# stefantaubert/waveglow

Measured on AMD Instinct MI355X. Metric: audio samples/sec/GPU (22.05 kHz) WaveGlow-256 infer; real-time factor, higher is better.
Workload: dtype f16 MFMA operands, f32 accumulate/flow state, fp16 I/O; 1 GPU; configs[1]: 256ch WaveGlow.infer, batch=16/GPU mels 80x864, fp16 I/O, sigma=0.6; parallelism=utterance-sharded x1, no collective

## Files before the change

### waveglow_amd/csrc/api.cpp

```cpp
#include <hip/hip_runtime.h>

#include <cmath>
#include <cstdarg>
#include <cstdio>
#include <cstdlib>
#include <cstring>
#include <map>
#include <string>
#include <vector>

#include "../../include/waveglow_amd.h"
#include "wg_common.h"

using namespace wg;

namespace {

thread_local std::string g_err;

int fail(int code, const char* fmt, ...) {
  char buf[512];
  va_list ap;
  va_start(ap, fmt);
  vsnprintf(buf, sizeof buf, fmt, ap);
// ... 57 lines not shown
constexpr float kSigmScale = -1.4426950408889634f;

struct LayerOffsets {
  size_t wA1, bias1, wA2, bias2, wEs;
  size_t wA1f = 0;
  size_t wA1x = 0, wA1fx = 0;
};
struct FlowOffsets {
  std::vector<LayerOffsets> layers;
  size_t wstart, bstart, out_init, winv, wfwd;
  size_t wStA = 0;
  int c, h;
  double logdet;
};

}

struct wg_handle {
  wg_config cfg;
  int device;
  int NS;
  std::vector<int> c_k;
  std::vector<std::string> expected;
  std::map<std::string, HostTensor> tensors;
  bool finalized = false;
  char* d_blob = nullptr;
  size_t blob_bytes = 0;
  char* d_cond = nullptr;
  char* d_cond16 = nullptr;
  size_t cond_layer_bytes = 0, cond_flow_bytes = 0;
  std::vector<FlowOffsets> flows;
  int n_cu = 256;
  int force_bn = 0;
  bool fold_start = true;
  unsigned long long* dbg_stamps = nullptr;
  bool prof = false;
  unsigned prof_mask = ~0u;
  std::vector<hipEvent_t> ev;
  std::vector<int> ev_class;
  size_t ev_used = 0;
  double prof_ms[8] = {0, 0, 0, 0, 0, 0, 0, 0};
  int64_t prof_n[8] = {0, 0, 0, 0, 0, 0, 0, 0};
  hipStream_t aux[3] = {nullptr, nullptr, nullptr};
  std::vector<hipEvent_t> sync_ev;
  size_t sync_next = 0;
  hipEvent_t mark_ev[16] = {nullptr, nullptr, nullptr, nullptr, nullptr, nullptr, nullptr, nullptr,
                            nullptr, nullptr, nullptr, nullptr, nullptr, nullptr, nullptr, nullptr};
  static constexpr int kPins = 4;
  void* pin[kPins] = {nullptr, nullptr, nullptr, nullptr};
  size_t pin_bytes[kPins] = {0, 0, 0, 0};
  hipEvent_t pin_ev[kPins] = {nullptr, nullptr, nullptr, nullptr};
  int pin_next = 0;
};

namespace {

std::vector<int> flow_channels(const wg_config& c) {
  std::vector<int> out;
  int rem = c.n_group;
  for (int k = 0; k < c.n_flows; ++k) {
    if (k % c.n_early_every == 0 && k > 0) rem -= c.n_early_size;
    out.push_back(rem);
  }
  return out;
}

// ... 147 lines not shown
}

extern "C" {

const char* wg_version(void) { return "waveglow_amd 0.1 (gfx950)"; }
const char* wg_last_error(void) { return g_err.c_str(); }

int wg_create(const wg_config* cfg, int device_id, wg_handle** out) {
  if (!cfg || !out) return fail(WG_ERR_INVALID, "null argument");
  const wg_config& c = *cfg;
  if (c.n_group != 8) return fail(WG_ERR_INVALID, "n_group=%d unsupported (only 8)", c.n_group);
  if (c.kernel_size != 3) return fail(WG_ERR_INVALID, "kernel_size=%d unsupported (only 3)", c.kernel_size);
  if (c.n_channels != 64 && c.n_channels != 128 && c.n_channels != 256 && c.n_channels != 512)
    return fail(WG_ERR_INVALID, "n_channels=%d unsupported (64, 128, 256, 512)", c.n_channels);
  if (c.n_layers < 1 || c.n_layers > 10) return fail(WG_ERR_INVALID, "n_layers=%d unsupported (1..10)", c.n_layers);
  if (c.upsample_kernel != 1024 || c.upsample_stride != 256)
    return fail(WG_ERR_INVALID, "upsample geometry %d/%d unsupported (1024/256)", c.upsample_kernel, c.upsample_stride);
  if (c.n_mel_channels < 16 || c.n_mel_channels > 80 || c.n_mel_channels % 16 != 0)
    return fail(WG_ERR_INVALID, "n_mel_channels=%d unsupported (multiple of 16, <= 80)", c.n_mel_channels);
  if (c.n_flows < 1 || c.n_early_every < 1 || c.n_early_size < 0 || c.n_early_size % 2 != 0)
    return fail(WG_ERR_INVALID, "bad flow configuration");
  std::vector<int> ck = flow_channels(c);
  if (ck.back() < 2 || ck.back() % 2 != 0) return fail(WG_ERR_INVALID, "flow configuration leaves %d channels", ck.back());
  wg_handle* h = new wg_handle();
  h->cfg = c;
  h->device = device_id;
  {
    int ncu = 0;
    if (hipDeviceGetAttribute(&ncu, hipDeviceAttributeMultiprocessorCount, device_id) == hipSuccess && ncu > 0) h->n_cu = ncu;
  }
  h->NS = c.n_mel_channels * c.n_group;
  h->c_k = ck;
  if (const char* e = getenv("WG_FORCE_BN")) h->force_bn = atoi(e);
  if (const char* e = getenv("WG_NO_START_FOLD")) h->fold_start = !(*e == '1');
  h->expected.push_back("upsample.weight");
  h->expected.push_back("upsample.bias");
  for (int k = 0; k < c.n_flows; ++k) {
    const std::string ks = std::to_string(k);
    h->expected.push_back("convinv." + ks + ".conv.weight");
    const std::string p = "WN." + ks + ".";
    for (const char* n : {"start", "cond_layer", "end"}) {
      h->expected.push_back(p + n + ".weight");
      h->expected.push_back(p + n + ".bias");
    }
    for (int i = 0; i < c.n_layers; ++i) {
      const std::string is = std::to_string(i);
      h->expected.push_back(p + "in_layers." + is + ".weight");
      h->expected.push_back(p + "in_layers." + is + ".bias");
      h->expected.push_back(p + "res_skip_layers." + is + ".weight");
      h->expected.push_back(p + "res_skip_layers." + is + ".bias");
    }
  }
  *out = h;
  return WG_OK;
}

int wg_destroy(wg_handle* h) {
  if (!h) return WG_OK;
  if (h->d_blob) hipFree(h->d_blob);
  if (h->d_cond) hipFree(h->d_cond);
  if (h->d_cond16) hipFree(h->d_cond16);
  for (hipEvent_t e : h->ev) hipEventDestroy(e);
  for (hipEvent_t e : h->sync_ev) hipEventDestroy(e);
  for (hipEvent_t e : h->mark_ev)
    if (e) hipEventDestroy(e);
  for (int i = 0; i < wg_handle::kPins; ++i) {
// ... 328 lines not shown
  return carve(h, g, nullptr).bytes;
}

size_t wg_forward_workspace_bytes(const wg_handle* h, int32_t B, int32_t n_frames, int32_t audio_len) {
  if (!h || B < 1 || n_frames < 1 || audio_len < h->cfg.n_group || audio_len % h->cfg.n_group) return 0;
  RowGeom g = make_geom(h->cfg, B, audio_len / h->cfg.n_group, n_frames);
  return carve(h, g, nullptr).bytes;
}

static int run_wn(wg_handle* h, int k, const RowGeom& g, Workspace& w, _Float16*& cur, _Float16*& oth, hipStream_t s) {
  const wg_config& c = h->cfg;
  const int C = c.n_channels;
  int BN = wn_block_n(C);
  if (BN == 128) {
    const int64_t t128 = (int64_t)kPhases * (g.Rp / 128), ncu = h->n_cu > 0 ? h->n_cu : 1;
    const int64_t r128 = (t128 + ncu - 1) / ncu, r64 = (2 * t128 + ncu - 1) / ncu;
    if (t128 < 4 * ncu && 6 * r64 < 10 * r128) BN = 64;
  }
  if (BN == 128 && h->force_bn == 64) BN = 64;
  if (h->force_bn == 128 && wn_block_n(C) == 128) BN = 128;
  const FlowOffsets& fo = h->flows[k];
  for (int i = 0; i < c.n_layers; ++i) {
    const LayerOffsets& lo = fo.layers[i];
    WnLayerArgs a;
    a.x_in = cur;
    a.x_out = oth;
    const bool fold0 = (i == 0) && h->fold_start;
    a.x_tap = fold0 ? w.A0 : cur;
    a.x_chunks_per_tap = fold0 ? 1 : C / 64;
    a.melT = w.melT;
    a.frag16 = wn_frag16(C, BN) ? 1 : 0;
    a.wStA = fold0 && wn_res_a0(C) ? (const _Float16*)(h->d_blob + fo.wStA) : nullptr;
    a.a0_fold = fold0 ? 1 : 0;
    a.wA1c = (const _Float16*)((a.frag16 ? h->d_cond16 : h->d_cond) + h->cond_flow_bytes * k + h->cond_layer_bytes * i);
    a.wA1 = (const _Float16*)(h->d_blob + (a.frag16 ? (fold0 ? lo.wA1fx : lo.wA1x) : (fold0 ? lo.wA1f : lo.wA1)));
    a.bias1 = (const float*)(h->d_blob + lo.bias1);
    a.wA2 = (const _Float16*)(h->d_blob + lo.wA2);
    a.bias2 = (const float*)(h->d_blob + lo.bias2);
    a.wEs = (const _Float16*)(h->d_blob + lo.wEs);
    a.out = w.OUT;
    a.g = g;
    a.dil = 1 << i;
    a.n_cond_steps = c.n_mel_channels / 16;
    a.M = c.n_mel_channels;
    a.has_res = i < c.n_layers - 1;
    a.row0 = 0;
    a.tiles_per_phase = g.Rp / BN;
    a.sp = nullptr;
    a.save_t = a.save_s = a.save_a = nullptr;
    a.in0 = a.in1 = nullptr;
    a.out0 = nullptr;
    a.n_tiles = kPhases * a.tiles_per_phase;
    a.stamps = h->dbg_stamps;
    a.n_cu = h->n_cu;
    {
      Prof p(h, s, 2);
      HIP_TRY(launch_wn_layer(a, C, BN, s));
    }
    WG_DBG(s, "wn_layer");
    if (a.has_res) std::swap(cur, oth);
  }
  return WG_OK;
}

int wg_infer(wg_handle* h, const void* mel, const void* z_init, const void* const* z_early, int32_t n_z_early,
             float sigma, void* audio, int32_t B, int32_t n_frames, int32_t io_dtype, void* workspace,
// ... 278 lines not shown
```

### waveglow_amd/csrc/kernels.hip

```cpp
#include "wg_common.h"

#include <cstdlib>
#include <type_traits>

namespace wg {

typedef _Float16 half8 __attribute__((ext_vector_type(8)));
typedef _Float16 half4 __attribute__((ext_vector_type(4)));
typedef float f32x16 __attribute__((ext_vector_type(16)));
typedef float f32x4 __attribute__((ext_vector_type(4)));

#define WG_GPTR(p) ((const __attribute__((address_space(1))) void*)(p))
#define WG_LPTR(p) ((__attribute__((address_space(3))) void*)(p))

__device__ __forceinline__ float load_io(const void* p, size_t i, int f16) {
  return f16 ? (float)((const _Float16*)p)[i] : ((const float*)p)[i];
}

__device__ __forceinline__ float gate_act(float u, float v) {
  const float e1 = __builtin_amdgcn_exp2f(__builtin_amdgcn_fmed3f(u, -60.0f, 60.0f));
  const float t = 1.0f + __builtin_amdgcn_exp2f(v);
  return (e1 - 1.0f) * __builtin_amdgcn_rcpf(fmaf(e1, t, t));
}

__device__ __forceinline__ void gate_act3(float u, float v, float& th, float& sg, float& ac) {
  const float e1 = __builtin_amdgcn_exp2f(__builtin_amdgcn_fmed3f(u, -60.0f, 60.0f));
  const float t = 1.0f + __builtin_amdgcn_exp2f(__builtin_amdgcn_fmed3f(v, -60.0f, 60.0f));
  const float r = __builtin_amdgcn_rcpf(fmaf(e1, t, t));
  ac = fmaf(e1, r, -r);
  sg = fmaf(e1, r, r);
  th = ac * t;
}

__device__ __forceinline__ void glds16(const void* sbase, unsigned voff, unsigned lds_addr) {
  unsigned keep;
  asm volatile("s_mov_b32 %0, m0\n\ts_mov_b32 m0, %3\n\ts_nop 2\n\tglobal_load_lds_dwordx4 %1, %2\n\ts_mov_b32 m0, %0"
               : "=&s"(keep) : "v"(voff), "s"(sbase), "s"(lds_addr) : "memory");
}
template <int OFF>
__device__ __forceinline__ void gload16(half8& dst, const void* sbase, unsigned voff) {
  asm volatile("s_nop 4\n\tglobal_load_dwordx4 %0, %1, %2 offset:%3" : "=v"(dst) : "v"(voff), "s"(sbase), "i"(OFF) : "memory");
}

#ifdef WG_STAMPS
#define WG_STAMP(i)                                                                              \
  do {                                                                                           \
    __builtin_amdgcn_sched_barrier(0);                                                           \
    unsigned long long _t;                                                                       \
    asm volatile("s_memtime %0\n\ts_waitcnt lgkmcnt(0)" : "=s"(_t)::"memory");                   \
    if (a.stamps && HAS_RES && tid == 0) a.stamps[(size_t)tile * 8 + (i)] = _t;                        \
    __builtin_amdgcn_sched_barrier(0);                                                           \
  } while (0)
#else
#define WG_STAMP(i) do {} while (0)
#endif

constexpr bool kPersistent = true;
#ifdef WG_DBG_NO_XTILE_DMA
constexpr bool kXTileDMA = false;
#else
constexpr bool kXTileDMA = kPersistent;
#endif
constexpr int kTilesPerWG = 2;
#ifdef WG_NO_PIPE_EPI
constexpr bool kPipeEpi = false;
#else
constexpr bool kPipeEpi = true;
#endif

#ifdef WG_NO_PRIO
constexpr bool kPrio = false;
#else
constexpr bool kPrio = true;
#endif
// ... 7 lines not shown
#else
constexpr bool kQ2Late = true;
#endif
#ifdef WG_NO_DEEP_Q2
constexpr bool kDeepQ2 = false;
#else
constexpr bool kDeepQ2 = true;
#endif
#ifdef WG_NO_WES_LDS
constexpr bool kWesLds = false;
#else
constexpr bool kWesLds = true;
#endif
#ifdef WG_NO_DEEP
constexpr bool kDeep = false;
#else
constexpr bool kDeep = true;
#endif

__device__ __forceinline__ void mfma16_acc(f32x4& c, const half8& a, const half8& b) {
  c = __builtin_amdgcn_mfma_f32_16x16x32_f16(a, b, c, 0, 0, 0);
}

template <int C> struct WnCfg {
  static constexpr int NW = (C >= 256) ? 8 : C / 32;
  static constexpr int BN = (C >= 512) ? 64 : 128;
};

template <int N> __device__ __forceinline__ void wait_vm() {
  asm volatile("s_waitcnt vmcnt(%0)" :: "i"(N) : "memory");
  __builtin_amdgcn_sched_barrier(0);
}

template <int C, int NW, int BN, bool HAS_RES, int TPW, int CX, int MODE = 0, int NTAPS = 3, bool HAS_COND = true, bool DEEP = false, bool M16 = false>
__global__ void __launch_bounds__(NW * 64) wn_layer_kernel(const WnLayerArgs a) {
  constexpr bool TR = MODE == 1;
  constexpr bool PLAIN = MODE >= 2;
  constexpr int MB = C / (32 * NW);
  constexpr int MT = PLAIN ? MB : 2 * MB;
  constexpr int NTHREADS = NW * 64;
  constexpr int NT = BN / 32;
  constexpr int CC = CX;
  constexpr int NKX = NTAPS * CC;
  constexpr int BT_BYTES = BN * 128;
  constexpr int ACT_ROW = 2 * C + 16;
  constexpr int K2 = C / 16;
  constexpr int NG = BN * 8 / NTHREADS;
  constexpr int NAH = MT * 2;
  constexpr bool DEFER = (MB == 1);
  static_assert(BN * 8 % NTHREADS == 0 && MB >= 1 && MB <= 2 && NKX >= 1 && (NTAPS == 1 || NTAPS == 3), "tile geometry");
  constexpr bool Q2L = !M16 && kQ2Late && DEFER && !DEEP && (NG + NT - 1) / NT == 1 && NT >= NG + MT;
  static_assert(!M16 || (MODE == 0 && MB == 1 && DEFER && !DEEP && NT >= 2), "16x16x32 variant");
  constexpr bool A0G = MODE == 0 && CX == 1 && NTAPS == 1;
  static_assert(!DEEP || (MODE == 0 && DEFER && HAS_COND && MT <= NT && NG <= NT && ((NKX >= 4 && NKX % 2 == 0) || NKX == 1)), "deep prefetch variant");
  static_assert(MODE == 0 || (TPW == 1 && CX == ((MODE == 2 || MODE == 4) ? 2 : 1) * (C / 64)) || (MODE == 3 && CX == 1), "training variants");

  extern __shared__ __attribute__((aligned(16))) char smem[];
  char* const sB = smem;
  char* const sActs = MODE == 4 ? smem : smem + 2 * BT_BYTES;

  const int tid = threadIdx.x;
  const int wave = __builtin_amdgcn_readfirstlane(tid >> 6);
  int lane = tid & 63, ln = lane & 31, lh = lane >> 5;

  unsigned pvoff[NG];
  int pchunk[NG];
  int swB;
  int l15 = lane & 15, l4 = lane >> 4;
  unsigned a_voff;
  auto set_lane_ids = [&]() {
    int t = tid;
    asm volatile("" : "+v"(t));
    lane = t & 63;
    ln = lane & 31;
    lh = lane >> 5;
    swB = M16 ? (lane >> 1) & 7 : (ln >> 1) & 7;
    l15 = lane & 15;
    l4 = lane >> 4;
    a_voff = lane * 16;
#pragma unroll
    for (int i = 0; i < NG; ++i) {
      const int idx = i * NTHREADS + t;
      const int row = idx >> 3, pc = idx & 7;
      pchunk[i] = pc ^ ((row >> 1) & 7);
      pvoff[i] = row * 128 + (pchunk[i] << 4);
    }
  };
  set_lane_ids();
  const unsigned sB_addr = (unsigned)(size_t)WG_LPTR(sB);
  const int R = a.g.R, Rp = a.g.Rp, Fp = a.g.Fp, M = a.M;
  const int nK = NKX + (HAS_COND ? a.n_cond_steps : 0);
  const int mel_rows_per_utt = a.g.T + 6;

  auto xstep_src = [&](int p, int jt, int ks) -> const char* {
    const int tap = ks / CC, cc = ks - tap * CC;
    const int pp = p + (tap - NTAPS / 2) * a.dil;
    const int row = kRowPad + (pp & 31) * Rp + a.row0 + jt * BN + (pp >> 5);
    return (const char*)(a.x_tap + ((size_t)cc * R + row) * 64);
  };
  auto sp_src = [&](int p, int jt, int s_) -> const char* {
    const int row = kRowPad + p * Rp + a.row0 + jt * BN;
    return (const char*)(a.sp + ((size_t)s_ * R + row) * 64);
  };
  int mrow[NG];
  auto cond_voff = [&](int s, int i) -> unsigned {
    const int k0 = s * 64 + pchunk[i] * 8;
    const int j = (k0 >= M) + (k0 >= 2 * M) + (k0 >= 3 * M);
    return (unsigned)(((mrow[i] - j) * M + (k0 - j * M)) * 2);
  };
  auto stage_B_piece = [&](int p, int jt, int ks, int bufsel, int i) {
#ifndef WG_DBG_NO_DMA
    const unsigned lds = __builtin_amdgcn_readfirstlane(sB_addr + bufsel * BT_BYTES + (i * NTHREADS + wave * 64) * 16);
    if constexpr (A0G) {
      if (ks < NKX) {
        const int row = (i * NTHREADS + tid) >> 3, lc = pchunk[i];
        const int pp = p + ((lc < 3 ? lc : 1) - 1) * a.dil;
        const unsigned prow = (unsigned)(kRowPad + (pp & 31) * Rp + a.row0 + jt * BN + (pp >> 5) + row);
        glds16(a.x_tap, prow * 128u + (lc < 3 ? 0u : (unsigned)lc * 16u), lds);
        return;
      }
    }
    if (ks < NKX) glds16(xstep_src(p, jt, ks), pvoff[i], lds);
    else if constexpr (MODE != 0) glds16(sp_src(p, jt, ks - NKX), pvoff[i], lds);
    else glds16(a.melT, cond_voff(ks - NKX, i), lds);
#endif
  };
  auto read_B = [&](const char* buf, int nt, int k16) -> half8 {
#ifdef WG_DBG_NO_LDSREAD
    half8 z; asm volatile("" : "=v"(z)); return z;
#endif
    const int n = nt * 32 + ln;
    const int c = (k16 * 2 + lh) ^ swB;
    return *(const half8*)(buf + n * 128 + c * 16);
  };
  auto read_B16 = [&](const char* buf, int g, int nt) -> half8 {
    const int n = (NT * (g & 1) + nt) * 16 + l15;
    const int c = (4 * (g >> 1) + l4) ^ swB;
    return *(const half8*)(buf + n * 128 + c * 16);
  };
  const char* wA1c_p = nullptr;
  auto load_Aq = [&](int ks, int g, int mt, half8& dst) {
    const char* base = ks < NKX ? (const char*)a.wA1 : wA1c_p;
    const int kl = ks < NKX ? ks : ks - NKX;
    const char* p = base + ((size_t)(2 * kl + (g >> 1)) * NW + wave) * (NAH * 1024) + (mt * 2 + (g & 1)) * 1024;
#ifndef WG_DBG_NO_ALOAD
    gload16<0>(dst, p, a_voff);
#else
    asm volatile("" : "=v"(dst));
#endif
  };
  auto load_A16 = [&](int ks, int s_, int m, half8& dst) {
    const char* base = ks < NKX ? (const char*)a.wA1 : wA1c_p;
    const int kl = ks < NKX ? ks : ks - NKX;
#ifndef WG_DBG_NO_ALOAD
    gload16<0>(dst, base + ((size_t)(2 * kl + s_) * NW + wave) * (NAH * 1024) + m * 1024, a_voff);
#else
    asm volatile("" : "=v"(dst));
#endif
  };
  int tile_b0 = 0;
  const bool fp_ge_bn = Fp >= BN;
  auto column_of = [&](int rr, int p, int& b, int& t) -> bool {
    int rem = rr - tile_b0 * Fp;
    b = tile_b0;
    if (fp_ge_bn) {
      if (rem >= Fp) { rem -= Fp; ++b; }
    } else {
      const int qd = rem / Fp;
      b += qd;
      rem -= qd * Fp;
    }
    const int fq = rem - a.g.Gf;
    t = fq * 32 + p;
    if (!(b < a.g.B && fq >= 0 && fq < a.g.F && t < a.g.L)) return false;
    return a.g.frames == nullptr || t < 32 * a.g.frames[b];
  };

  int tile, tile_end;
  const int tile_step = gridDim.x >> 3;
  int run_start, run_quarter = 0;
  {
    const int bid = blockIdx.x, ntl = a.n_tiles;
    const int xcd = bid & 7, idx = bid >> 3;
    const int qq = ntl >> 3, r = ntl & 7;
    const int start = xcd < r ? xcd * (qq + 1) : r * (qq + 1) + (xcd - r) * qq;
    tile_end = start + (xcd < r ? qq + 1 : qq);
    tile = start + idx;
    run_start = start;
// ... 23 lines not shown
#pragma unroll
  for (int it = 0; it < TPW; ++it, tile += tile_step) {
    if (tile >= tile_end) break;
    if (it > 0) set_lane_ids();
    const int tile_m = tile_of(tile);
    const int p = tile_m / a.tiles_per_phase;
    const int jt = tile_m - p * a.tiles_per_phase;
    const int rr0 = a.row0 + jt * BN;
    tile_b0 = rr0 / Fp;
    const int r0 = kRowPad + p * Rp + rr0;
    const int next_tile = tile + tile_step;
    wA1c_p = (const char*)a.wA1c + (MODE != 0 ? (size_t)0 : (size_t)p * (2 * a.n_cond_steps) * NW * (NAH * 1024));
    if constexpr (!kXTileDMA) {
      if (it > 0) {
#pragma unroll
        for (int i = 0; i < NG; ++i) stage_B_piece(p, jt, 0, par, i);
      }
    }
    half8 Q[DEEP ? 2 : 1][4][MT];
    if constexpr (DEEP) {
#pragma unroll
      for (int g = 0; g < 4; ++g)
#pragma unroll
        for (int mt = 0; mt < MT; ++mt) load_Aq(0, g, mt, Q[0][g][mt]);
#pragma unroll
      for (int g = 0; g < (kDeepQ2 ? 2 : 3); ++g)
#pragma unroll
        for (int mt = 0; mt < MT; ++mt) load_Aq(1, g, mt, Q[DEEP ? 1 : 0][g][mt]);
    } else {
#pragma unroll
      for (int g = 0; g < (Q2L || M16 ? 2 : 3); ++g)
#pragma unroll
        for (int mt = 0; mt < MT; ++mt) {
          if constexpr (M16) load_A16(0, 0, 2 * g + mt, q[g][mt]);
          else load_Aq(0, g, mt, q[g][mt]);
        }
    }
    if constexpr (MODE == 0) {
#pragma unroll
      for (int i = 0; i < NG; ++i) {
        int b, t;
        const int rr = rr0 + ((i * NTHREADS + tid) >> 3);
        const bool ok = column_of(rr, p, b, t);
        mrow[i] = ok ? 3 + b * mel_rows_per_utt + 3 + (t >> 5) : 3;
      }
    }
    unsigned vmask = 0;
#pragma unroll
    for (int nt = 0; nt < NT; ++nt) {
      int cb, ct;
      vmask |= column_of(rr0 + nt * 32 + ln, p, cb, ct) ? (1u << nt) : 0u;
    }
    WG_STAMP(0);
    f32x16 acc[MT][NT];
    f32x4 acc4[M16 ? MT : 1][M16 ? NT : 1][4];
    auto acc_at = [&](int mt, int nt, int e) -> float {
      if constexpr (M16) return acc4[mt][nt][e >> 2][e & 3];
      else return acc[mt][nt][e];
    };
#pragma unroll
    for (int mt = 0; mt < MT; ++mt) {
      f32x16 v;
      if constexpr (PLAIN) {
#pragma unroll
        for (int j = 0; j < 16; ++j) v[j] = 0.0f;
      } else {
        const int row0 = (mt < MB ? 0 : C) + (wave * MB + (mt < MB ? mt : mt - MB)) * 32;
// ... 25 lines not shown
    constexpr int LPS = (MT + NT - 1) / NT;
    constexpr int GPS = (NG + NT - 1) / NT;
    half8 bf[2][NT];
    constexpr bool PRIO = kPrio && NW == 8 && ((BN == 128 && ((MODE == 0 && CX == C / 64) || MODE == 1)) || (C == 512 && MODE == 0 && CX == C / 64));
    auto prio_set = [&](int hi_grp) {
      if (hi_grp == 1)
        asm volatile("s_cmp_lt_u32 %0, 4\n\ts_cbranch_scc1 .Lpa%=\n\ts_setprio 1\n\ts_branch .Lpb%=\n.Lpa%=:\n\ts_setprio 0\n.Lpb%=:" :: "s"(wave) : "memory", "scc");
      else
        asm volatile("s_cmp_lt_u32 %0, 4\n\ts_cbranch_scc1 .Lpa%=\n\ts_setprio 0\n\ts_branch .Lpb%=\n.Lpa%=:\n\ts_setprio 1\n.Lpb%=:" :: "s"(wave) : "memory", "scc");
    };
    auto mfma_col = [&](int g, int nt) {
      if constexpr (M16) {
        const int t16 = NT * (g & 1) + nt;
#pragma unroll
        for (int m = 0; m < 4; ++m) {
          mfma16_acc(acc4[m >> 1][t16 >> 1][2 * (m & 1) + (t16 & 1)], q[2 * (g >> 1) + (m >> 1)][m & 1], bf[g & 1][nt]);
        }
      } else {
#pragma unroll
        for (int mt = 0; mt < MT; ++mt) {
#ifdef WG_DBG_MFMA16
          f32x4 lo = __builtin_shufflevector(acc[mt][nt], acc[mt][nt], 0, 1, 2, 3);
          f32x4 hi = __builtin_shufflevector(acc[mt][nt], acc[mt][nt], 4, 5, 6, 7);
          lo = __builtin_amdgcn_mfma_f32_16x16x32_f16(q[g][mt], bf[g & 1][nt], lo, 0, 0, 0);
          hi = __builtin_amdgcn_mfma_f32_16x16x32_f16(q[g][mt], bf[g & 1][nt], hi, 0, 0, 0);
#pragma unroll
          for (int j = 0; j < 4; ++j) { acc[mt][nt][j] = lo[j]; acc[mt][nt][4 + j] = hi[j]; }
#else
          acc[mt][nt] = __builtin_amdgcn_mfma_f32_32x32x16_f16(q[g][mt], bf[g & 1][nt], acc[mt][nt], 0, 0, 0);
#endif
        }
      }
    };
    auto kstep = [&](auto more_tag, auto ncond_tag, auto first_tag, int ks) {
      constexpr bool more = decltype(more_tag)::value;
      constexpr bool ncond = decltype(ncond_tag)::value;
      constexpr bool first = decltype(first_tag)::value;
      const char* buf = sB + ((ks + par) & 1) * BT_BYTES;
      const char* src_next = nullptr;
      if constexpr (more && !ncond) src_next = xstep_src(p, jt, ks + 1);
      if constexpr (more && ncond && MODE != 0) src_next = sp_src(p, jt, ks + 1 - NKX);
      const unsigned lds_next = sB_addr + ((ks + 1 + par) & 1) * BT_BYTES + wave * 1024;
#pragma unroll
      for (int nt = 0; nt < NT; ++nt) bf[0][nt] = M16 ? read_B16(buf, 0, nt) : read_B(buf, nt, 0);
      __builtin_amdgcn_sched_barrier(0);
      auto dma_slot = [&](int nt) {
        if constexpr (more) {
#pragma unroll
          for (int i = nt * GPS; i < (nt + 1) * GPS && i < NG; ++i) {
#ifndef WG_DBG_NO_DMA
            const unsigned lds = __builtin_amdgcn_readfirstlane(lds_next + i * NTHREADS * 16);
            if constexpr (ncond && MODE == 0) glds16(a.melT, cond_voff(ks + 1 - NKX, i), lds);
            else glds16(src_next, pvoff[i], lds);
#endif
          }
        }
      };
      if constexpr (PRIO) {
        prio_set(1);
        __builtin_amdgcn_sched_barrier(0);
      }
      if constexpr (DEFER) {
#pragma unroll
        for (int nt = 0; nt < NT; ++nt) {
          if constexpr (!first) mfma_col(3, nt);
          __builtin_amdgcn_sched_barrier(0);
          dma_slot(nt);
          if constexpr (Q2L) {
            if (nt >= NG && nt - NG < MT) load_Aq(ks, 2, nt - NG, q[2][nt - NG]);
          }
          __builtin_amdgcn_sched_barrier(0);
        }
      }
#pragma unroll
      for (int g = 0; g < (DEFER ? 3 : 4); ++g) {
        if constexpr (M16) {
          if (g == 0) wait_vm<more ? NG : 0>();
          if (g == 2) wait_vm<0>();
        } else {
        if (g == 1) wait_vm<more ? 2 * MT + NG : 2 * MT>();
        if (g == 2) wait_vm<Q2L ? (more ? 2 * MT : MT) : (more ? NG + 2 * MT : MT)>();
        if (g == 3) wait_vm<more ? 2 * MT : 0>();
        }
#pragma unroll
        for (int nt = 0; nt < NT; ++nt) {
          mfma_col(g, nt);
          __builtin_amdgcn_sched_barrier(0);
          if (g < 3) bf[(g + 1) & 1][nt] = M16 ? read_B16(buf, g + 1, nt) : read_B(buf, nt, g + 1);
          if (!DEFER && g == 0) dma_slot(nt);
          if constexpr (M16) {
            constexpr int LP16 = (4 + NT - 1) / NT;
            if (g == 0 || (g == 2 && more)) {
#pragma unroll
              for (int m = nt * LP16; m < (nt + 1) * LP16 && m < 4; ++m)
                load_A16(g == 0 ? ks : ks + 1, g == 0 ? 1 : 0, m, q[(g == 0 ? 2 : 0) + (m >> 1)][m & 1]);
            }
          } else if (g == 0 || more) {
#pragma unroll
            for (int mt = nt * LPS; mt < (nt + 1) * LPS && mt < MT; ++mt)
              load_Aq(g == 0 ? ks : ks + 1, (g + 3) & 3, mt, q[(g + 3) & 3][mt]);
          }
          if constexpr (PRIO) {
            if (g == 0 && nt == NT - 1) prio_set(0);
          }
          __builtin_amdgcn_sched_barrier(0);
        }
      }
      if constexpr (more) {
        if constexpr (DEFER && !Q2L && !M16) {
#pragma unroll
          for (int mt = 0; mt < MT; ++mt) load_Aq(ks + 1, 2, mt, q[2][mt]);
        }
        asm volatile("s_waitcnt vmcnt(%0) lgkmcnt(0)" :: "i"(M16 ? 4 : Q2L ? MT : 2 * MT) : "memory");
#ifndef WG_DBG_NO_BARRIER
        __builtin_amdgcn_s_barrier();
#endif
        __builtin_amdgcn_sched_barrier(0);
      }
    };
    auto kstep_d = [&](auto par_tag, auto more_tag, auto more2_tag, auto ncond_tag, auto first_tag, int ks) {
      constexpr int P = DEEP ? decltype(par_tag)::value : 0, PO = DEEP ? 1 - P : 0;
      constexpr bool more = decltype(more_tag)::value, more2 = decltype(more2_tag)::value;
      constexpr bool ncond = decltype(ncond_tag)::value, first = decltype(first_tag)::value;
      const char* buf = sB + ((ks + par) & 1) * BT_BYTES;
      const char* src_next = nullptr;
      if constexpr (more && !ncond) src_next = xstep_src(p, jt, ks + 1);
      const unsigned lds_next = sB_addr + ((ks + 1 + par) & 1) * BT_BYTES + wave * 1024;
#pragma unroll
// ... 55 lines not shown
      using P1 = std::integral_constant<int, 1>;
      if constexpr (NKX == 1) {
        kstep_d(P0{}, T_{}, T_{}, T_{}, T_{}, 0);
        kstep_d(P1{}, T_{}, T_{}, T_{}, F_{}, 1);
        kstep_d(P0{}, T_{}, T_{}, T_{}, F_{}, 2);
        kstep_d(P1{}, T_{}, T_{}, T_{}, F_{}, 3);
        kstep_d(P0{}, T_{}, F_{}, T_{}, F_{}, 4);
        kstep_d(P1{}, F_{}, F_{}, F_{}, F_{}, 5);
      } else {
        kstep_d(P0{}, T_{}, T_{}, F_{}, T_{}, 0);
#pragma clang loop unroll(disable)
        for (int ks = 1; ks < NKX - 1; ks += 2) {
          kstep_d(P1{}, T_{}, T_{}, F_{}, F_{}, ks);
          kstep_d(P0{}, T_{}, T_{}, F_{}, F_{}, ks + 1);
        }
        kstep_d(P1{}, T_{}, T_{}, T_{}, F_{}, NKX - 1);
        kstep_d(P0{}, T_{}, T_{}, T_{}, F_{}, NKX);
        kstep_d(P1{}, T_{}, T_{}, T_{}, F_{}, NKX + 1);
        kstep_d(P0{}, T_{}, T_{}, T_{}, F_{}, NKX + 2);
        kstep_d(P1{}, T_{}, F_{}, T_{}, F_{}, NKX + 3);
        kstep_d(P0{}, F_{}, F_{}, F_{}, F_{}, NKX + 4);
      }
      constexpr int PL = (NKX + 4) & 1;
      wait_vm<0>();
#pragma unroll
      for (int nt = 0; nt < NT; ++nt)
#pragma unroll
        for (int mt = 0; mt < MT; ++mt)
          acc[mt][nt] = __builtin_amdgcn_mfma_f32_32x32x16_f16(Q[DEEP ? PL : 0][3][mt], bf[1][nt], acc[mt][nt], 0, 0, 0);
    }
    if constexpr (!DEEP) {
      using T_ = std::true_type;
      using F_ = std::false_type;
      if constexpr (NKX == 1) {
        if constexpr (HAS_COND) kstep(T_{}, T_{}, T_{}, 0);
        else kstep(F_{}, F_{}, T_{}, 0);
      } else {
        kstep(T_{}, F_{}, T_{}, 0);
#pragma clang loop unroll(disable)
        for (int ks = 1; ks < NKX - 1; ++ks) kstep(T_{}, F_{}, F_{}, ks);
        if constexpr (HAS_COND) kstep(T_{}, T_{}, F_{}, NKX - 1);
        else kstep(F_{}, F_{}, F_{}, NKX - 1);
      }
      if constexpr (HAS_COND) {
#pragma clang loop unroll(disable)
        for (int ks = NKX; ks < nK - 1; ++ks) kstep(T_{}, T_{}, F_{}, ks);
        kstep(F_{}, F_{}, F_{}, nK - 1);
      }
    }
    if constexpr (DEFER && !DEEP) {
      wait_vm<0>();
#pragma unroll
      for (int nt = 0; nt < NT; ++nt) mfma_col(3, nt);
    }
    if constexpr (PRIO) asm volatile("s_setprio 0" ::: "memory");
    __builtin_amdgcn_sched_barrier(0);
    par = (par + nK) & 1;
    if constexpr (kXTileDMA) {
      if (next_tile < tile_end) {
        const int tn = tile_of(next_tile), pn = tn / a.tiles_per_phase;
#pragma unroll
        for (int i = 0; i < NG; ++i) stage_B_piece(pn, tn - pn * a.tiles_per_phase, 0, par, i);
      }
    }
    __builtin_amdgcn_sched_barrier(0);

    WG_STAMP(2);
    if constexpr (PLAIN) {
      auto gate_derivative = [&](const f32x16& g, const _Float16* tp, const _Float16* sp_, _Float16* dst, size_t off) {
        const half8 t0 = *(const half8*)(tp + off), t1 = *(const half8*)(tp + off + 8);
        const half8 s0 = *(const half8*)(sp_ + off), s1 = *(const half8*)(sp_ + off + 8);
        half8 o0, o1, p0, p1;
#pragma unroll
        for (int r = 0; r < 8; ++r) {
          const float ta = (float)t0[r], sa = (float)s0[r], ga = g[r];
          const float tb = (float)t1[r], sb = (float)s1[r], gb = g[8 + r];
          o0[r] = (_Float16)(ga * sa * (1.0f - ta * ta));
          o1[r] = (_Float16)(gb * sb * (1.0f - tb * tb));
          p0[r] = (_Float16)(ga * ta * sa * (1.0f - sa));
          p1[r] = (_Float16)(gb * tb * sb * (1.0f - sb));
// ... 465 lines not shown
      if constexpr (!kWesEarly) es_prefetch();
      es_compute();
    }

    if constexpr (!PIPE) WG_STAMP(5);
    if constexpr (HAS_RES && !PIPE) {
#pragma unroll
      for (int nt = 0; nt < NT; ++nt) {
        int cb, ct;
        if (column_of(rr0 + nt * 32 + lno, p, cb, ct)) {
#pragma unroll
          for (int mb = 0; mb < MB; ++mb) {
            const int blk = wave * MB + mb;
            half8 o0, o1;
#pragma unroll
            for (int r = 0; r < 8; ++r) {
              o0[r] = (_Float16)acc2[mb][nt][r];
              o1[r] = (_Float16)acc2[mb][nt][8 + r];
            }
            const size_t row = (size_t)(blk >> 1) * R + r0 + nt * 32 + lno;
            half8* xp = (half8*)(a.x_out + row * 64 + (blk & 1) * 32 + lho * 16);
            xp[0] = o0;
            xp[1] = o1;
          }
        }
      }
    }
    if constexpr (!PIPE) WG_STAMP(6);
    }
    __builtin_amdgcn_sched_barrier(0);
  }
}

template <int C, int BN, bool HAS_RES, int TPW, int CX, int MODE = 0, int NTAPS = 3, bool HAS_COND = true, bool DEEP = false>
static hipError_t launch_wn_tttt(const WnLayerArgs& a, hipStream_t s) {
  constexpr int NW = WnCfg<C>::NW;
  constexpr bool M16 = wn_frag16(C, BN) && MODE == 0 && !DEEP;
  if (M16 != (a.frag16 != 0)) return hipErrorInvalidValue;
  if (MODE == 0 && CX == 1 && NTAPS == 1 && wn_res_a0(C) && HAS_RES && !a.wStA) return hipErrorInvalidValue;
  constexpr int smem = MODE == 4 ? (BN * (2 * C + 16) > 2 * BN * 128 ? BN * (2 * C + 16) : 2 * BN * 128)
                                 : 2 * BN * 128 + (MODE >= 2 ? 0 : BN * (2 * C + 16) + 3 * C * 4 + (kWesLds ? (C / 32) * 1024 : 0));
  static bool attr_done_dev[64] = {};
  int cur_dev = 0;
  if (hipGetDevice(&cur_dev) != hipSuccess || cur_dev < 0 || cur_dev >= 64) cur_dev = 0;
  bool& attr_done = attr_done_dev[cur_dev];
  if (!attr_done) {
    hipError_t e = hipFuncSetAttribute((const void*)wn_layer_kernel<C, NW, BN, HAS_RES, TPW, CX, MODE, NTAPS, HAS_COND, DEEP, M16>,
                                       hipFuncAttributeMaxDynamicSharedMemorySize, smem);
    if (e != hipSuccess) return e;
    attr_done = true;
  }
  const int per_label = ((a.n_tiles + 7) / 8 + TPW - 1) / TPW;
  const int grid = 8 * per_label;
  hipLaunchKernelGGL((wn_layer_kernel<C, NW, BN, HAS_RES, TPW, CX, MODE, NTAPS, HAS_COND, DEEP, M16>), dim3(grid), dim3(NW * 64), smem, s, a);
  return hipGetLastError();
}
template <int C, int BN, bool HAS_RES, int TPW>
static hipError_t launch_wn_ttt(const WnLayerArgs& a, hipStream_t s) {
  if constexpr (kDeep && C == 256 && BN == 64 && TPW == 1) {
    const char* e = getenv("WG_DISABLE_DEEP");
    if (a.n_cond_steps == 5 && !(e && *e == '1')) {
      if (a.a0_fold) return launch_wn_tttt<C, BN, HAS_RES, TPW, 1, 0, 1, true, true>(a, s);
      return launch_wn_tttt<C, BN, HAS_RES, TPW, C / 64, 0, 3, true, true>(a, s);
    }
  }
  if (a.a0_fold) return a.x_chunks_per_tap == 1 ? launch_wn_tttt<C, BN, HAS_RES, TPW, 1, 0, 1>(a, s) : hipErrorInvalidValue;
  return launch_wn_tttt<C, BN, HAS_RES, TPW, C / 64>(a, s);
}
template <int C, int BN, bool HAS_RES>
static hipError_t launch_wn_tt(const WnLayerArgs& a, hipStream_t s) {
  const int ncu = a.n_cu > 0 ? a.n_cu : 1;
  const int rounds1 = (a.n_tiles + ncu - 1) / ncu;
  const int rounds2 = ((a.n_tiles + kTilesPerWG - 1) / kTilesPerWG + ncu - 1) / ncu * kTilesPerWG;
  if (a.n_tiles >= 2 * kTilesPerWG * ncu && rounds2 <= rounds1) return launch_wn_ttt<C, BN, HAS_RES, kTilesPerWG>(a, s);
  return launch_wn_ttt<C, BN, HAS_RES, 1>(a, s);
}
template <int C>
static hipError_t launch_wn_t(const WnLayerArgs& a, int bn, hipStream_t s) {
  if (bn == 64) return a.has_res ? launch_wn_tt<C, 64, true>(a, s) : launch_wn_tt<C, 64, false>(a, s);
  if constexpr (WnCfg<C>::BN == 128) {
    if (bn == 128) return a.has_res ? launch_wn_tt<C, 128, true>(a, s) : launch_wn_tt<C, 128, false>(a, s);
  }
  return hipErrorInvalidValue;
}

int wn_block_n(int C) {
  switch (C) {
    case 64: return WnCfg<64>::BN;
    case 128: return WnCfg<128>::BN;
    case 256: return WnCfg<256>::BN;
    case 512: return WnCfg<512>::BN;
  }
  return 0;
}
int wn_waves(int C) {
  switch (C) {
    case 64: return WnCfg<64>::NW;
    case 128: return WnCfg<128>::NW;
    case 256: return WnCfg<256>::NW;
// ... 418 lines not shown
```

### waveglow_amd/csrc/wg_common.h

```cpp
#pragma once
#include <hip/hip_runtime.h>
#include <stdint.h>

namespace wg {

__host__ __device__ inline int pos_to_chan(int P) {
  const int blk = P >> 5, p = P & 31;
  const int h = p >> 4, g = (p >> 2) & 3, i = p & 3;
  return (blk << 5) + 8 * g + 4 * h + i;
}
__host__ __device__ inline int chan_to_pos(int c) {
  const int blk = c >> 5, o = c & 31;
  const int g = o >> 3, h = (o >> 2) & 1, i = o & 3;
  return (blk << 5) + 16 * h + 4 * g + i;
}

constexpr int kMaxGroup = 8;
constexpr int kBK = 64;

struct RowGeom {
  int B;
  int L;
  int F;
  int Gf;
// ... 11 lines not shown
constexpr int kPhases = 32;

#ifdef WG_NO_M16
constexpr bool wn_frag16(int, int) { return false; }
#else
constexpr bool wn_frag16(int C, int BN) { return C == 256 && BN == 128; }
#endif

constexpr bool wn_res_a0(int) { return true; }

struct WnLayerArgs {
  const _Float16* x_in;
  const _Float16* x_tap;
  int x_chunks_per_tap;
  _Float16* x_out;
  const _Float16* melT;
  const _Float16* wA1;
  const _Float16* wA1c;
  const float* bias1;
  const _Float16* wA2;
  const float* bias2;
  const _Float16* wEs;
  float* out;
  RowGeom g;
  int dil;
  int n_cond_steps;
  int M;
  int has_res;
  int row0;
  int tiles_per_phase;
  int n_tiles;
  int n_cu;
  int frag16 = 0;
  int a0_fold = 0;
  const _Float16* wStA = nullptr;
  unsigned long long* stamps;
  const _Float16* sp;
  _Float16* save_t;
  _Float16* save_s;
  _Float16* save_a;
  const _Float16* in0;
  const _Float16* in1;
  _Float16* out0;
  const _Float16* wat_prev;
  const _Float16* gout;
  const _Float16* t_prev;
  const _Float16* s_prev;
  _Float16* dpre_prev;
};

struct MelPackArgs {
  const int* frames;
  const void* mel;
  _Float16* melT;
  int B, M, T, io_f16;
};

struct FlowArgs {
  int direction;
  int first;
  int c_in;
  int h_in;
  const float* winv;
  const void* z_extra;
  int n_extra;
  float sigma;
// ... 41 lines not shown
```

Before: 78.99 million samples/s.

## Share staged input windows across dilated taps in WN layers

For 256-channel WN layers with dilation 32-128, the kernel now stages each channel chunk's input rows once into an extended LDS window (held in the activation buffer), plus a few tail rows. The three dilated taps then read shifted views of that window with an adjusted swizzle instead of DMAing each tap separately. This cuts global-to-LDS traffic for later k-steps. It also drops the s_nop padding before A-weight loads in the steady-state steps. It adds LDS pressure, a new kernel variant and more complex wait counts.

```diff
diff --git a/waveglow_amd/csrc/api.cpp b/waveglow_amd/csrc/api.cpp
--- a/waveglow_amd/csrc/api.cpp
+++ b/waveglow_amd/csrc/api.cpp
@@ -113,6 +113,7 @@
   std::vector<FlowOffsets> flows;
   int n_cu = 256;
   int force_bn = 0;
+  bool tap_share = true;
   bool fold_start = true;
   unsigned long long* dbg_stamps = nullptr;
   bool prof = false;
@@ -326,6 +327,7 @@
   h->NS = c.n_mel_channels * c.n_group;
   h->c_k = ck;
   if (const char* e = getenv("WG_FORCE_BN")) h->force_bn = atoi(e);
+  if (const char* e = getenv("WG_NO_TAP_SHARE")) h->tap_share = !(*e == '1');
   if (const char* e = getenv("WG_NO_START_FOLD")) h->fold_start = !(*e == '1');
   h->expected.push_back("upsample.weight");
   h->expected.push_back("upsample.bias");
@@ -720,6 +722,7 @@
     a.frag16 = wn_frag16(C, BN) ? 1 : 0;
     a.wStA = fold0 && wn_res_a0(C) ? (const _Float16*)(h->d_blob + fo.wStA) : nullptr;
     a.a0_fold = fold0 ? 1 : 0;
+    a.tap_share = h->tap_share ? 1 : 0;
     a.wA1c = (const _Float16*)((a.frag16 ? h->d_cond16 : h->d_cond) + h->cond_flow_bytes * k + h->cond_layer_bytes * i);
     a.wA1 = (const _Float16*)(h->d_blob + (a.frag16 ? (fold0 ? lo.wA1fx : lo.wA1x) : (fold0 ? lo.wA1f : lo.wA1)));
     a.bias1 = (const float*)(h->d_blob + lo.bias1);
diff --git a/waveglow_amd/csrc/kernels.hip b/waveglow_amd/csrc/kernels.hip
--- a/waveglow_amd/csrc/kernels.hip
+++ b/waveglow_amd/csrc/kernels.hip
@@ -40,6 +40,10 @@
 template <int OFF>
 __device__ __forceinline__ void gload16(half8& dst, const void* sbase, unsigned voff) {
   asm volatile("s_nop 4\n\tglobal_load_dwordx4 %0, %1, %2 offset:%3" : "=v"(dst) : "v"(voff), "s"(sbase), "i"(OFF) : "memory");
+}
+template <int OFF>
+__device__ __forceinline__ void gload16_ss(half8& dst, const void* sbase, unsigned voff) {
+  asm volatile("global_load_dwordx4 %0, %1, %2 offset:%3" : "=v"(dst) : "v"(voff), "s"(sbase), "i"(OFF) : "memory");
 }
 
 #ifdef WG_STAMPS
@@ -113,7 +117,7 @@
   __builtin_amdgcn_sched_barrier(0);
 }
 
-template <int C, int NW, int BN, bool HAS_RES, int TPW, int CX, int MODE = 0, int NTAPS = 3, bool HAS_COND = true, bool DEEP = false, bool M16 = false>
+template <int C, int NW, int BN, bool HAS_RES, int TPW, int CX, int MODE = 0, int NTAPS = 3, bool HAS_COND = true, bool DEEP = false, bool M16 = false, int SH = 0>
 __global__ void __launch_bounds__(NW * 64) wn_layer_kernel(const WnLayerArgs a) {
   constexpr bool TR = MODE == 1;
   constexpr bool PLAIN = MODE >= 2;
@@ -133,6 +137,9 @@
   constexpr bool Q2L = !M16 && kQ2Late && DEFER && !DEEP && (NG + NT - 1) / NT == 1 && NT >= NG + MT;
   static_assert(!M16 || (MODE == 0 && MB == 1 && DEFER && !DEEP && NT >= 2), "16x16x32 variant");
   constexpr bool A0G = MODE == 0 && CX == 1 && NTAPS == 1;
+  constexpr bool SHARE = SH != 0;
+  constexpr int WIN_BYTES = (BN + 8) * 128;
+  static_assert(!SHARE || (M16 && NTAPS == 3 && CC == 4 && NG < NT && 1024 + 3 * WIN_BYTES <= BN * ACT_ROW), "shared tap staging");
   static_assert(!DEEP || (MODE == 0 && DEFER && HAS_COND && MT <= NT && NG <= NT && ((NKX >= 4 && NKX % 2 == 0) || NKX == 1)), "deep prefetch variant");
   static_assert(MODE == 0 || (TPW == 1 && CX == ((MODE == 2 || MODE == 4) ? 2 : 1) * (C / 64)) || (MODE == 3 && CX == 1), "training variants");
 
@@ -149,6 +156,7 @@
   int swB;
   int l15 = lane & 15, l4 = lane >> 4;
   unsigned a_voff;
+  const int sh = SHARE ? a.dil >> 5 : 0;
   auto set_lane_ids = [&]() {
     int t = tid;
     asm volatile("" : "+v"(t));
@@ -214,9 +222,9 @@
     const int c = (k16 * 2 + lh) ^ swB;
     return *(const half8*)(buf + n * 128 + c * 16);
   };
-  auto read_B16 = [&](const char* buf, int g, int nt) -> half8 {
+  auto read_B16 = [&](const char* buf, int g, int nt, int sw) -> half8 {
     const int n = (NT * (g & 1) + nt) * 16 + l15;
-    const int c = (4 * (g >> 1) + l4) ^ swB;
+    const int c = (4 * (g >> 1) + l4) ^ sw;
     return *(const half8*)(buf + n * 128 + c * 16);
   };
   const char* wA1c_p = nullptr;
@@ -230,11 +238,13 @@
     asm volatile("" : "=v"(dst));
 #endif
   };
-  auto load_A16 = [&](int ks, int s_, int m, half8& dst) {
+  auto load_A16 = [&](int ks, int s_, int m, half8& dst, auto ss_tag) {
     const char* base = ks < NKX ? (const char*)a.wA1 : wA1c_p;
     const int kl = ks < NKX ? ks : ks - NKX;
 #ifndef WG_DBG_NO_ALOAD
-    gload16<0>(dst, base + ((size_t)(2 * kl + s_) * NW + wave) * (NAH * 1024) + m * 1024, a_voff);
+    const char* src = base + ((size_t)(2 * kl + s_) * NW + wave) * (NAH * 1024) + m * 1024;
+    if constexpr (decltype(ss_tag)::value) gload16_ss<0>(dst, src, a_voff);
+    else gload16<0>(dst, src, a_voff);
 #else
     asm volatile("" : "=v"(dst));
 #endif
@@ -324,7 +334,7 @@
       for (int g = 0; g < (Q2L || M16 ? 2 : 3); ++g)
 #pragma unroll
         for (int mt = 0; mt < MT; ++mt) {
-          if constexpr (M16) load_A16(0, 0, 2 * g + mt, q[g][mt]);
+          if constexpr (M16) load_A16(0, 0, 2 * g + mt, q[g][mt], std::false_type{});
           else load_Aq(0, g, mt, q[g][mt]);
         }
     }
@@ -416,20 +426,46 @@
         }
       }
     };
-    auto kstep = [&](auto more_tag, auto ncond_tag, auto first_tag, int ks) {
+    const unsigned sActs_addr = (unsigned)(size_t)WG_LPTR(sActs);
+    auto win_addr = [&](int cc) -> unsigned {
+      return cc == 0 ? sB_addr + par * BT_BYTES : sActs_addr + 1024 + (cc - 1) * WIN_BYTES;
+    };
+    auto kstep = [&](auto more_tag, auto ncond_tag, auto first_tag, auto dk_tag, auto ss_tag, int ks) {
       constexpr bool more = decltype(more_tag)::value;
       constexpr bool ncond = decltype(ncond_tag)::value;
       constexpr bool first = decltype(first_tag)::value;
+      constexpr int dk = decltype(dk_tag)::value;
+      constexpr bool dma = more && (!SHARE || ncond || dk >= 1);
+      constexpr bool tails = SHARE && more && !ncond && dk == 2;
+      constexpr int NDMA = (dma ? NG : 0) + (tails ? 1 : 0);
       const char* buf = sB + ((ks + par) & 1) * BT_BYTES;
+      int swk = swB;
+      if constexpr (SHARE) {
+        if (ks < NKX) {
+          const int tap = ks >> 2;
+          const int cc = ks & 3;
+          buf = (cc == 0 ? sB + par * BT_BYTES : sActs + 1024 + (cc - 1) * WIN_BYTES) + tap * sh * 128;
+          swk = ((l15 + tap * sh) >> 1) & 7;
+        }
+      }
       const char* src_next = nullptr;
       if constexpr (more && !ncond) src_next = xstep_src(p, jt, ks + 1);
       if constexpr (more && ncond && MODE != 0) src_next = sp_src(p, jt, ks + 1 - NKX);
-      const unsigned lds_next = sB_addr + ((ks + 1 + par) & 1) * BT_BYTES + wave * 1024;
-#pragma unroll
-      for (int nt = 0; nt < NT; ++nt) bf[0][nt] = M16 ? read_B16(buf, 0, nt) : read_B(buf, nt, 0);
+      const unsigned lds_next = (SHARE && !ncond ? win_addr(ks + 1) : sB_addr + ((ks + 1 + par) & 1) * BT_BYTES) + wave * 1024;
+#pragma unroll
+      for (int nt = 0; nt < NT; ++nt) bf[0][nt] = M16 ? read_B16(buf, 0, nt, swk) : read_B(buf, nt, 0);
       __builtin_amdgcn_sched_barrier(0);
       auto dma_slot = [&](int nt) {
-        if constexpr (more) {
+        if constexpr (tails) {
+          if (nt == NG) {
+            const int cc = wave & 3;
+            const unsigned lds = __builtin_amdgcn_readfirstlane(win_addr(cc) + BN * 128);
+            const int tr = (tid >> 3) & 7;
+            const int sr = tr < 2 * sh ? tr : 2 * sh - 1;
+            glds16(xstep_src(p, jt, cc), (unsigned)((BN + sr) * 128 + (((tid & 7) ^ (((BN + tr) >> 1) & 7)) << 4)), lds);
+          }
+        }
+        if constexpr (dma) {
 #pragma unroll
           for (int i = nt * GPS; i < (nt + 1) * GPS && i < NG; ++i) {
 #ifndef WG_DBG_NO_DMA
@@ -459,7 +495,7 @@
 #pragma unroll
       for (int g = 0; g < (DEFER ? 3 : 4); ++g) {
         if constexpr (M16) {
-          if (g == 0) wait_vm<more ? NG : 0>();
+          if (g == 0) wait_vm<NDMA>();
           if (g == 2) wait_vm<0>();
         } else {
         if (g == 1) wait_vm<more ? 2 * MT + NG : 2 * MT>();
@@ -470,14 +506,14 @@
         for (int nt = 0; nt < NT; ++nt) {
           mfma_col(g, nt);
           __builtin_amdgcn_sched_barrier(0);
-          if (g < 3) bf[(g + 1) & 1][nt] = M16 ? read_B16(buf, g + 1, nt) : read_B(buf, nt, g + 1);
+          if (g < 3) bf[(g + 1) & 1][nt] = M16 ? read_B16(buf, g + 1, nt, swk) : read_B(buf, nt, g + 1);
           if (!DEFER && g == 0) dma_slot(nt);
           if constexpr (M16) {
             constexpr int LP16 = (4 + NT - 1) / NT;
             if (g == 0 || (g == 2 && more)) {
 #pragma unroll
               for (int m = nt * LP16; m < (nt + 1) * LP16 && m < 4; ++m)
-                load_A16(g == 0 ? ks : ks + 1, g == 0 ? 1 : 0, m, q[(g == 0 ? 2 : 0) + (m >> 1)][m & 1]);
+                load_A16(g == 0 ? ks : ks + 1, g == 0 ? 1 : 0, m, q[(g == 0 ? 2 : 0) + (m >> 1)][m & 1], ss_tag);
             }
           } else if (g == 0 || more) {
 #pragma unroll
@@ -599,20 +635,30 @@
     if constexpr (!DEEP) {
       using T_ = std::true_type;
       using F_ = std::false_type;
+      using D0 = std::integral_constant<int, 0>;
+      using D1 = std::integral_constant<int, 1>;
+      using D2 = std::integral_constant<int, 2>;
       if constexpr (NKX == 1) {
-        if constexpr (HAS_COND) kstep(T_{}, T_{}, T_{}, 0);
-        else kstep(F_{}, F_{}, T_{}, 0);
+        if constexpr (HAS_COND) kstep(T_{}, T_{}, T_{}, D1{}, F_{}, 0);
+        else kstep(F_{}, F_{}, T_{}, D1{}, F_{}, 0);
+      } else if constexpr (SHARE) {
+        kstep(T_{}, F_{}, T_{}, D2{}, F_{}, 0);
+#pragma clang loop unroll(disable)
+        for (int ks = 1; ks < 3; ++ks) kstep(T_{}, F_{}, F_{}, D1{}, T_{}, ks);
+#pragma clang loop unroll(disable)
+        for (int ks = 3; ks < NKX - 1; ++ks) kstep(T_{}, F_{}, F_{}, D0{}, T_{}, ks);
+        kstep(T_{}, T_{}, F_{}, D1{}, F_{}, NKX - 1);
       } else {
-        kstep(T_{}, F_{}, T_{}, 0);
+        kstep(T_{}, F_{}, T_{}, D1{}, F_{}, 0);
 #pragma clang loop unroll(disable)
-        for (int ks = 1; ks < NKX - 1; ++ks) kstep(T_{}, F_{}, F_{}, ks);
-        if constexpr (HAS_COND) kstep(T_{}, T_{}, F_{}, NKX - 1);
-        else kstep(F_{}, F_{}, F_{}, NKX - 1);
+        for (int ks = 1; ks < NKX - 1; ++ks) kstep(T_{}, F_{}, F_{}, D1{}, T_{}, ks);
+        if constexpr (HAS_COND) kstep(T_{}, T_{}, F_{}, D1{}, F_{}, NKX - 1);
+        else kstep(F_{}, F_{}, F_{}, D1{}, F_{}, NKX - 1);
       }
       if constexpr (HAS_COND) {
 #pragma clang loop unroll(disable)
-        for (int ks = NKX; ks < nK - 1; ++ks) kstep(T_{}, T_{}, F_{}, ks);
-        kstep(F_{}, F_{}, F_{}, nK - 1);
+        for (int ks = NKX; ks < nK - 1; ++ks) kstep(T_{}, T_{}, F_{}, D1{}, T_{}, ks);
+        kstep(F_{}, F_{}, F_{}, D1{}, F_{}, nK - 1);
       }
     }
     if constexpr (DEFER && !DEEP) {
@@ -1144,7 +1190,7 @@
   }
 }
 
-template <int C, int BN, bool HAS_RES, int TPW, int CX, int MODE = 0, int NTAPS = 3, bool HAS_COND = true, bool DEEP = false>
+template <int C, int BN, bool HAS_RES, int TPW, int CX, int MODE = 0, int NTAPS = 3, bool HAS_COND = true, bool DEEP = false, int SH = 0>
 static hipError_t launch_wn_tttt(const WnLayerArgs& a, hipStream_t s) {
   constexpr int NW = WnCfg<C>::NW;
   constexpr bool M16 = wn_frag16(C, BN) && MODE == 0 && !DEEP;
@@ -1157,14 +1203,14 @@
   if (hipGetDevice(&cur_dev) != hipSuccess || cur_dev < 0 || cur_dev >= 64) cur_dev = 0;
   bool& attr_done = attr_done_dev[cur_dev];
   if (!attr_done) {
-    hipError_t e = hipFuncSetAttribute((const void*)wn_layer_kernel<C, NW, BN, HAS_RES, TPW, CX, MODE, NTAPS, HAS_COND, DEEP, M16>,
+    hipError_t e = hipFuncSetAttribute((const void*)wn_layer_kernel<C, NW, BN, HAS_RES, TPW, CX, MODE, NTAPS, HAS_COND, DEEP, M16, SH>,
                                        hipFuncAttributeMaxDynamicSharedMemorySize, smem);
     if (e != hipSuccess) return e;
     attr_done = true;
   }
   const int per_label = ((a.n_tiles + 7) / 8 + TPW - 1) / TPW;
   const int grid = 8 * per_label;
-  hipLaunchKernelGGL((wn_layer_kernel<C, NW, BN, HAS_RES, TPW, CX, MODE, NTAPS, HAS_COND, DEEP, M16>), dim3(grid), dim3(NW * 64), smem, s, a);
+  hipLaunchKernelGGL((wn_layer_kernel<C, NW, BN, HAS_RES, TPW, CX, MODE, NTAPS, HAS_COND, DEEP, M16, SH>), dim3(grid), dim3(NW * 64), smem, s, a);
   return hipGetLastError();
 }
 template <int C, int BN, bool HAS_RES, int TPW>
@@ -1177,6 +1223,10 @@
     }
   }
   if (a.a0_fold) return a.x_chunks_per_tap == 1 ? launch_wn_tttt<C, BN, HAS_RES, TPW, 1, 0, 1>(a, s) : hipErrorInvalidValue;
+  if constexpr (wn_frag16(C, BN) && C / 64 == 4 && TPW == 1) {
+    if (a.tap_share && a.dil >= 32 && a.dil <= 128 && a.dil % 32 == 0 && a.x_chunks_per_tap == C / 64)
+      return launch_wn_tttt<C, BN, HAS_RES, TPW, C / 64, 0, 3, true, false, 1>(a, s);
+  }
   return launch_wn_tttt<C, BN, HAS_RES, TPW, C / 64>(a, s);
 }
 template <int C, int BN, bool HAS_RES>
diff --git a/waveglow_amd/csrc/wg_common.h b/waveglow_amd/csrc/wg_common.h
--- a/waveglow_amd/csrc/wg_common.h
+++ b/waveglow_amd/csrc/wg_common.h
@@ -67,6 +67,7 @@
   int n_tiles;
   int n_cu;
   int frag16 = 0;
+  int tap_share = 0;
   int a0_fold = 0;
   const _Float16* wStA = nullptr;
   unsigned long long* stamps;
```

Result: no change. 79.47 million samples/s (median of 6 runs) (+0.6%).
